# rubengooj/pl-slam

Measured on AMD Instinct MI355X. Metric: stereo pairs/sec (1500 ORB + 200 LBD BF-match), higher is better.
Workload: dtype fp4; 1 GPU; C2: synthetic 752x480 stereo stream, 1500 ORB + 200 LBD per image, ORB+LBD L<->R and prev<->curr, mutual + ratio (StVO::match), then StereoFrame's gates over the L<->R tables (config_kitti.yaml:25-...; mutual=True, distinct_batches_in_rotation=3, stereo_gates=True, kernel=k_scan_sym_mfma_i, mfma_form=0

## Files before the change

plslam_amd/csrc/hamming_mfma_i.hip:

```cpp
#include "mfma_h_common.hpp"

#include <type_traits>


namespace plslam {

namespace {
constexpr uint32_t MI_MAG = FP4_FOUR;
constexpr int MI_DSHIFT = 5;
constexpr uint32_t MI_ACC_BITS = 0x4B000000u + 4096u;
constexpr uint32_t MI_KEY16_MAX = 0x3FFFu;
constexpr uint32_t MI_COL_PENALTY = 0x4000u;
constexpr int MI_SCALE_A = 0, MI_SCALE_B = 0;
constexpr uint32_t MI_NONE16 = 0x7BFFu;
constexpr uint32_t MI_NONE32 = MI_NONE16 * 0x00010001u;
constexpr int MI_RESCAN_BATCH = 2;
constexpr int MI_RESCAN_BATCH16 = 2;
constexpr int MI_VGPRS = 168;
}

#ifdef PLSLAM_MI_PROF
constexpr int MI_PROF_WGS = 65536;
__device__ unsigned long long g_mi_prof[MI_PROF_WGS * 4];
#define PLSLAM_MI_TICK() __builtin_readcyclecounter()
#endif

template <bool DIRECTED>
__global__ void __launch_bounds__(256, 3) __attribute__((amdgpu_num_vgpr(MI_VGPRS / 2)))
k_scan_sym_mfma_i(const SymDesc* __restrict__ syms, const BlockDesc* __restrict__ blocks, int32_t* __restrict__ zero, int nzero, int nblocks)
{
    constexpr int ROWX_STRIDE = 33;
    constexpr int MI_ROW_STRIDE = MH_ROW_STRIDE, MI_TILE_BYTES = MH_TILE_N * MI_ROW_STRIDE;
    constexpr int PARK_OFF = 2 * MI_TILE_BYTES;
    constexpr int SMEM_BYTES = PARK_OFF + 4 * 16 * 64 * 8;
    static_assert(SMEM_BYTES >= 4 * 64 * ROWX_STRIDE * 4, "the transpose must fit");
    __shared__ __attribute__((aligned(16))) uint8_t smem[SMEM_BYTES];
    __shared__ __attribute__((aligned(16))) uint32_t colstage[MH_CGROUP * 256];
    constexpr int RING = 3;
    __shared__ __attribute__((aligned(16))) uint32_t rawring[RING][256];
    uint8_t* const btile = smem;
    u32x2_t* const park = reinterpret_cast<u32x2_t*>(smem + PARK_OFF) + (threadIdx.x >> 6) * (16 * 64) + (threadIdx.x & 63);

#ifdef PLSLAM_MI_PROF
    const unsigned long long prof_t0 = PLSLAM_MI_TICK();
    unsigned long long prof_loop = 0, prof_fin = 0, prof_tl = 0;
#endif
    if (blockIdx.x == 0)
        for (int i = threadIdx.x; i < nzero; i += 256) zero[i] = 0;
    asm volatile("s_setreg_imm32_b32 hwreg(HW_REG_MODE, 6, 2), 3");

    (void)nblocks;
    const int wg = xcd_remap_(blockIdx.x, gridDim.x);
    const BlockDesc bd = blocks[wg];
    if (bd.item < 0) return;
    const SymDesc sd = syms[bd.item];
    const int n1 = sd.n1, n2 = sd.n2;
    const MhLayout L(n2);
    const int ntiles = L.ntiles, nfull = L.nfull, rag_s = L.rag_s;
    const int n2p = (MH_TILE_N * ntiles + 255) & ~255;
    const int tid = threadIdx.x, lane = tid & 63;
    const int w = __builtin_amdgcn_readfirstlane(tid >> 6);
    const int c = lane & 31, g = lane >> 5;
    const gcu32_t araw = (gcu32_t) reinterpret_cast<const uint32_t*>(sd.a);
    const int iw = bd.row0 + 32 * w;

    i32x4 afrag[2][MH_KSTEPS];

    uint32_t gm[16];
#pragma unroll
    for (int s = 0; s < 16; ++s) gm[s] = MI_NONE32;

    u32x16 seed;
#pragma unroll
    for (int r = 0; r < 16; ++r) seed[r] = MI_ACC_BITS + (uint32_t)(16 * g + r);
    asm volatile("" : "+v"(seed));
    const int rest = n2 - (nfull >> 4) * MH_GROUP_ROWS;
    auto lane_lim = [&]() __attribute__((always_inline)) -> int {
        const int cc = (int)(threadIdx.x & 31u), v = rest - rag_s * cc;
        return rag_s == 0 ? 0 : (v < 0 ? 0 : (v > rag_s ? rag_s : v));
    };
    const int lim_part = rag_s ? rest % rag_s : 0;
    const int mask_from = rest - 31 * rag_s < 0 ? 0 : rest - 31 * rag_s;

    const bool block_ragged = bd.row0 + 256 > n1;
    const bool wide_part = !DIRECTED && (sd.flags & 1);
    const gu32_t part = DIRECTED ? (gu32_t) nullptr : (gu32_t) sd.part21 + (size_t)(bd.row0 >> 8) * n2p * (wide_part ? 2 : 1);
    uint32_t* const cstage = colstage + 64 * w;
#pragma unroll
    for (int k = 0; k < 2; ++k) *reinterpret_cast<i32x4*>(colstage + 8 * tid + 4 * k) = i32x4{-1, -1, -1, -1};

    const int ej = tid >> 3, ewd4 = (tid & 7) * 4;
    const PLSLAM_GLOBAL char* const bbytes = (const PLSLAM_GLOBAL char*) sd.b;
    auto load_raw = [&](int t) __attribute__((always_inline)) -> uint32_t {
        const int tc = t < ntiles ? t : ntiles - 1;
        const int gbase = (tc >> 4) * MH_GROUP_ROWS;
        const uint32_t s = tc < nfull ? (uint32_t)MH_GROUP : (uint32_t)rag_s;
        uint32_t row = __umul24((uint32_t)ej, s) + (uint32_t)(tc & 15);
        const uint32_t last = (uint32_t)(n2 - 1 - gbase);
        row = row < last ? row : last;
        return *reinterpret_cast<gcu32_t>(bbytes + (size_t)gbase * 32 + (row * 32u + (uint32_t)ewd4));
    };
    auto load_raw_async = [&](int t, uint32_t slot_b) __attribute__((always_inline)) {
        const int tc = t < ntiles ? t : ntiles - 1;
        const uint32_t s = tc < nfull ? (uint32_t)MH_GROUP : (uint32_t)rag_s;
        const uint32_t first = ((uint32_t)(tc & ~15) << 5) + (uint32_t)(tc & 15);
        uint32_t row = __umul24((uint32_t)ej, s) + first;
        const uint32_t last = (uint32_t)(n2 - 1);
        row = row < last ? row : last;
        const uint32_t voff = row * 32u + (uint32_t)ewd4;
        const uint32_t lds_dst = (uint32_t)(uintptr_t)(&rawring[0][64 * w]) + slot_b;
        asm volatile("s_mov_b32 m0, %2\n\ts_nop 0\n\tglobal_load_lds_dword %0, %1" : : "v"(voff), "s"(bbytes), "s"(lds_dst) : "memory", "m0");
    };
    uint32_t pf32 = 0;
    auto load_raw_async_full = [&](uint32_t slot_b) __attribute__((always_inline)) {
        const uint32_t voff = (uint32_t)(ej * (MH_GROUP * 32) + ewd4) + pf32;
        const uint32_t lds_dst = (uint32_t)(uintptr_t)(&rawring[0][64 * w]) + slot_b;
        asm volatile("s_mov_b32 m0, %2\n\ts_nop 0\n\tglobal_load_lds_dword %0, %1" : : "v"(voff), "s"(bbytes), "s"(lds_dst) : "memory", "m0");
    };
    auto take_raw = [&](uint32_t slot_b) __attribute__((always_inline)) -> uint32_t {
        asm volatile("s_waitcnt vmcnt(2)" ::: "memory");
        return *reinterpret_cast<const uint32_t*>(reinterpret_cast<const uint8_t*>(&rawring[0][0]) + slot_b + (ej * 32 + ewd4));
    };
    auto expand_store = [&](uint32_t raw, int buf, int tn, bool full = false) __attribute__((always_inline)) {
        uint8_t* dst = btile + buf * MI_TILE_BYTES + ej * MI_ROW_STRIDE + ewd4 * 4;
        i32x4 v = expand_dword_fp4<false, MI_MAG>(raw);
        if (!full && tn >= nfull && (tn & 15) >= mask_from) {
            const int vm = (int)(__umul24((uint32_t)rag_s, (uint32_t)ej) + (uint32_t)(tn & 15)) < rest ? -1 : 0;
            v &= i32x4{vm, vm, vm, vm};
        }
        *reinterpret_cast<i32x4*>(dst) = v;
    };

    int wt0 = 0, wt1 = ntiles < MH_WINDOW ? ntiles : MH_WINDOW;
    uint32_t ring_slot = 1024;

    const uint64_t part_u = (uint64_t)(uintptr_t)part;
    const uint64_t part_s = ((uint64_t)(uint32_t)__builtin_amdgcn_readfirstlane((int)(part_u >> 32)) << 32) |
                            (uint32_t)__builtin_amdgcn_readfirstlane((int)(uint32_t)part_u);
    auto combine_columns = [&](int kb) __attribute__((always_inline)) {
        if (DIRECTED) return;
        uint32_t l_;
        asm volatile("v_mbcnt_lo_u32_b32 %0, -1, 0\n\tv_mbcnt_hi_u32_b32 %0, -1, %0" : "=&v"(l_));
        const uint32_t* const src = colstage + 512 * w + (((l_ & 32u) << 3) | (l_ & 31u));
        uint32_t p[8];
#pragma unroll
        for (int v = 0; v < 4; ++v) { p[2 * v] = src[64 * v]; p[2 * v + 1] = src[64 * v + 32]; }
        if (block_ragged) {
#pragma unroll
            for (int q = 0; q < 8; ++q) {
                const int base = bd.row0 + 32 * (q >> 1) + 16 * (q & 1);
                const uint32_t strike = (base >= n1 ? MI_NONE16 : 0u) | (base + 128 >= n1 ? MI_NONE16 << 16 : 0u);
                p[q] = pk_max16(p[q], strike);
            }
        }
        auto pk_merge = [](uint32_t& a0, uint32_t& a1, uint32_t c0, uint32_t c1) {
            const uint32_t m = pk_max16(a0, c0);
            a0 = pk_min16(a0, c0);
            a1 = pk_min16(m, pk_min16(a1, c1));
        };
        uint32_t k0, k1;
        if (!wide_part) {
            uint32_t lo[4], hi[4], enc[4];
#pragma unroll
            for (int q = 0; q < 4; ++q) { lo[q] = pk_min16(p[2 * q], p[2 * q + 1]); hi[q] = pk_max16(p[2 * q], p[2 * q + 1]); }
#pragma unroll
            for (int q = 0; q < 4; ++q) {
                uint32_t t;
                asm("v_pk_add_u16 %0, %1, %2" : "=v"(t) : "v"(lo[q]), "v"((uint32_t)(32 * q) * 0x00010001u));
                asm("v_pk_mad_u16 %0, %1, %2, %3 clamp" : "=v"(enc[q]) : "v"(lo[q] & 0xFFE0FFE0u), "v"(0x00030003u), "v"(t));
            }
            const uint32_t best = pk_min16(pk_min16(enc[0], enc[1]), pk_min16(enc[2], enc[3]));
            pk_merge(lo[0], hi[0], lo[1], hi[1]);
            pk_merge(lo[2], hi[2], lo[3], hi[3]);
            pk_merge(lo[0], hi[0], lo[2], hi[2]);
            const uint32_t e0 = best & 0xFFFFu, u0 = best >> 16, e1 = hi[0] & 0xFFE0u, u1 = (hi[0] >> 16) & 0xFFE0u;
            k0 = e0 + (e0 & 0xFF80u);
            k1 = e1 << 3;
            merge2(k0, k1, u0 + (u0 & 0xFF80u) + 128u, u1 << 3);
        } else {
#pragma unroll
            for (int q = 0; q < 8; ++q) {
                const uint32_t t = p[q] & 0x001F001Fu;
                uint32_t sh;
                asm("v_pk_lshlrev_b16 %0, %1, %2" : "=v"(sh) : "v"(0x00020002u), "v"(p[q] & 0xFFE0FFE0u));
                p[q] = sh | t | ((uint32_t)(q >> 1) << 5) * 0x00010001u;
            }
            uint32_t lo[4], hi[4];
#pragma unroll
            for (int q = 0; q < 4; ++q) { lo[q] = pk_min16(p[2 * q], p[2 * q + 1]); hi[q] = pk_max16(p[2 * q], p[2 * q + 1]); }
            pk_merge(lo[0], hi[0], lo[1], hi[1]);
            pk_merge(lo[2], hi[2], lo[3], hi[3]);
            pk_merge(lo[0], hi[0], lo[2], hi[2]);
            const uint32_t e0 = lo[0] & 0xFFFFu, e1 = hi[0] & 0xFFFFu, u0 = lo[0] >> 16, u1 = hi[0] >> 16;
            k0 = e0 + (e0 & 0xFF80u); k1 = e1 + (e1 & 0xFF80u);
            merge2(k0, k1, u0 + (u0 & 0xFF80u) + 128u, u1 + (u1 & 0xFF80u) + 128u);
        }
        const uint32_t slot4 = (uint32_t)(256 * kb + 64 * w) * 4u;
        if (!wide_part) {
            const uint32_t e = (umin_(k0, 0x1FFFFu) << 9) | umin_(k1 >> 8, 511u);
            PLSLAM_GLOBAL uint32_t* dst = (PLSLAM_GLOBAL uint32_t*)((PLSLAM_GLOBAL char*)(uintptr_t)(part_s + slot4) + 4u * l_);
            __builtin_nontemporal_store(e, dst);
        } else {
            const u32x2_t e = {k0, k1};
            PLSLAM_GLOBAL u32x2_t* dst = (PLSLAM_GLOBAL u32x2_t*)((PLSLAM_GLOBAL char*)(uintptr_t)(part_s + 2u * slot4) + 8u * l_);
            __builtin_nontemporal_store(e, dst);
        }
    };
    auto push_groups = [&gm, &wt0, &park](int t, auto final_tag, u32x2_t* rb) __attribute__((always_inline)) {
        constexpr bool FINAL = decltype(final_tag)::value;
        const uint32_t grp = (uint32_t)(((t - wt0) >> 4) & 3);
        const uint32_t gtag = grp * 0x00010001u;
        uint32_t gtv = gtag;
        asm volatile("" : "+v"(gtv));
        auto retag = [&](uint32_t x) -> uint32_t {
            uint32_t r;
            asm("v_and_or_b32 %0, %1, %2, %3" : "=v"(r) : "v"(x), "s"(0xFFE0FFE0u), "v"(gtv));
            return r;
        };
        if (grp == 0) {
#pragma unroll
            for (int s = 0; s < 16; ++s) {
                const u32x2_t v = {retag(gm[s]), 0xFFFFFFFFu};
                if (FINAL) rb[s] = v;
                else park[s * 64] = v;
                gm[s] = MI_NONE32;
            }
            return;
        }
#pragma unroll
        for (int s = 0; s < 16; ++s) {
            const u32x2_t v = park[s * 64];
            uint32_t b0 = v.x, b1 = v.y;
            pk_push2(b0, b1, retag(gm[s]));
            if (FINAL) rb[s] = u32x2_t{b0, b1};
            else park[s * 64] = u32x2_t{b0, b1};
            gm[s] = MI_NONE32;
        }
    };
    auto finish_columns = [&](int t, uint32_t c0, uint32_t c1) __attribute__((always_inline)) {
        if (DIRECTED) { asm volatile("" ::"v"(c0), "v"(c1)); return; }
        cstage[(t & (MH_CGROUP - 1)) * 256 + lane] = __builtin_amdgcn_perm(c1, c0, 0x05040100u);
    };

#define PLSLAM_MI_EPI2(ACC, MT, Q)                                                                 \
    {                                                                                              \
        asm("v_pk_minimum3_f16 %0, %0, %1, %2 op_sel:[0,0,1] op_sel_hi:[1,1,0]" : "+v"(gm[8 * (MT) + (Q)]) : "v"(ACC[Q]), "v"(ACC[(Q) + 8])); \
        asm("v_pk_minimum3_f16 %0, %0, %1, %2 op_sel:[0,0,1] op_sel_hi:[1,1,0]" : "+v"(gm[8 * (MT) + (Q) + 1]) : "v"(ACC[(Q) + 1]), "v"(ACC[(Q) + 9])); \
        if (!DIRECTED) {    \
            if ((Q) == 0) asm("v_min_f32 %0, %1, %2" : "=v"(cfa) : "v"(ACC[Q]), "v"(ACC[(Q) + 8])); \
            else asm("v_min3_f32 %0, %0, %1, %2" : "+v"(cfa) : "v"(ACC[Q]), "v"(ACC[(Q) + 8]));    \
            asm("v_min3_f32 %0, %0, %1, %2" : "+v"(cfa) : "v"(ACC[(Q) + 1]), "v"(ACC[(Q) + 9]));   \
        }                                                                                          \
        __builtin_amdgcn_sched_barrier(0);                                                         \
    }
#define PLSLAM_MI_MMA(ACC, MT, KS, CIN)                                                            \
    {                                                                                              \
        const i32x8 a8 = {afrag[MT][KS].x, afrag[MT][KS].y, afrag[MT][KS].z, afrag[MT][KS].w, 0, 0, 0, 0}; \
        const i32x8 b8 = {bfr[KS].x, bfr[KS].y, bfr[KS].z, bfr[KS].w, 0, 0, 0, 0};                 \
        ACC = __builtin_amdgcn_mfma_scale_f32_32x32x64_f8f6f4(a8, b8, CIN, 4, 4, 0, MI_SCALE_A, 0, MI_SCALE_B); \
        asm volatile("" : "+v"(ACC));                      \
        __builtin_amdgcn_sched_barrier(0);                                                         \
    }
    f32x16 m1;
    uint32_t cm0_prev = MI_NONE32;
    auto tile_step = [&](int t, auto u_tag, bool with_prev, auto full_tag) __attribute__((always_inline)) {
        constexpr bool FULL = decltype(full_tag)::value;
        constexpr int U = decltype(u_tag)::value;
        __syncthreads();
        const uint8_t* bt = btile + (U & 1) * MI_TILE_BYTES + c * MI_ROW_STRIDE + 16 * g;
        i32x4 bfr[MH_KSTEPS];
#define PLSLAM_MI_READ_B(KS) (*reinterpret_cast<const i32x4*>(bt + 32 * (KS)))
        bfr[0] = PLSLAM_MI_READ_B(0);
        bfr[1] = PLSLAM_MI_READ_B(1);
        if (!FULL && t >= nfull && ((t & 15) == 0 || (t & 15) == lim_part)) {
            const uint32_t pen = lane_lim() == (t & 15) ? MI_COL_PENALTY : 0u;
#pragma unroll
            for (int r = 0; r < 16; ++r) seed[r] += pen;
            asm volatile("" : "+v"(seed));
        }
        const f32x16 cseed = __builtin_bit_cast(f32x16, seed);
        f32x16 m0;
        float cfa = 0.0f;
        auto cf_join = [&]() __attribute__((always_inline)) -> uint32_t { return __builtin_bit_cast(uint32_t, cfa); };
        __builtin_amdgcn_sched_barrier(0);
        if (DIRECTED) asm volatile("s_nop 7"); else asm volatile("s_nop 4");
        __builtin_amdgcn_sched_barrier(0);
        PLSLAM_MI_EPI2(m1, 1, 0) PLSLAM_MI_MMA(m0, 0, 0, cseed)
        bfr[2] = PLSLAM_MI_READ_B(2);
        PLSLAM_MI_EPI2(m1, 1, 2) PLSLAM_MI_MMA(m0, 0, 1, m0)
        bfr[3] = PLSLAM_MI_READ_B(3);
        PLSLAM_MI_EPI2(m1, 1, 4) PLSLAM_MI_MMA(m0, 0, 2, m0)
        const uint32_t raw_next = take_raw(ring_slot);
        PLSLAM_MI_EPI2(m1, 1, 6) PLSLAM_MI_MMA(m0, 0, 3, m0)
        const uint32_t cm1 = cf_join();
        expand_store(raw_next, (U + 1) & 1, t + 1, FULL);
        if (FULL) {
            load_raw_async_full(ring_slot);
            pf32 += (U == 3 && ((t + 5) & 15) == 0) ? (MH_GROUP_ROWS - 15) * 32u : 32u;
        } else {
            load_raw_async(t + 4, ring_slot);
        }
        ring_slot = ring_slot == 2048u ? 0u : ring_slot + 1024u;
        if (with_prev) {
            if (!DIRECTED && U == 1 && ((t - 1) & (MH_CGROUP - 1)) == 0 && t - 9 >= wt0) {
                combine_columns((t - 9) >> 3);
                __syncthreads();
            }
            finish_columns(t - 1, cm0_prev, cm1);
            if (U == 0 && ((t - 1) & (MH_GROUP - 1)) == MH_GROUP - 1) push_groups(t - 1, std::false_type{}, nullptr);
        }
        __builtin_amdgcn_sched_barrier(0);
        asm volatile("v_mfma_f32_32x32x64_f8f6f4 %0, %1, %2, %3 cbsz:4 blgp:4" : "=&v"(m1) : "v"(afrag[1][0]), "v"(bfr[0]), "v"(cseed));
        __builtin_amdgcn_sched_barrier(0);
        PLSLAM_MI_EPI2(m0, 0, 0)
        PLSLAM_MI_MMA(m1, 1, 1, m1)    PLSLAM_MI_EPI2(m0, 0, 2)
        PLSLAM_MI_MMA(m1, 1, 2, m1)    PLSLAM_MI_EPI2(m0, 0, 4)
        PLSLAM_MI_MMA(m1, 1, 3, m1)    PLSLAM_MI_EPI2(m0, 0, 6)
        cm0_prev = cf_join();
    };
    auto epilogue = [&](int t) __attribute__((always_inline)) {
        float cfa = 0.0f;
        asm volatile("s_nop 7\n\ts_nop 7");
        __builtin_amdgcn_sched_barrier(0);
        PLSLAM_MI_EPI2(m1, 1, 0) PLSLAM_MI_EPI2(m1, 1, 2) PLSLAM_MI_EPI2(m1, 1, 4) PLSLAM_MI_EPI2(m1, 1, 6)
        finish_columns(t, cm0_prev, __builtin_bit_cast(uint32_t, cfa));
    };
    auto pipeline = [&](u32x2_t* rb) __attribute__((always_inline)) {
        {
            u32x16 none;
#pragma unroll
            for (int r = 0; r < 16; ++r) asm volatile("v_mov_b32 %0, %1" : "=v"(none[r]) : "s"(MI_NONE32));
            m1 = __builtin_bit_cast(f32x16, none);
        }
        int tb = wt0;
        {
            const int lim = (wt1 < nfull ? wt1 : nfull) - 7;
            pf32 = (((uint32_t)((tb + 4) & ~15) << 5) + (uint32_t)((tb + 4) & 15)) * 32u;
            for (; tb < lim; tb += 4) {
                tile_step(tb, std::integral_constant<int, 0>{}, tb != wt0, std::true_type{});
                tile_step(tb + 1, std::integral_constant<int, 1>{}, true, std::true_type{});
                tile_step(tb + 2, std::integral_constant<int, 2>{}, true, std::true_type{});
                tile_step(tb + 3, std::integral_constant<int, 3>{}, true, std::true_type{});
            }
        }
        for (; tb < wt1; tb += 4) {
            tile_step(tb, std::integral_constant<int, 0>{}, tb != wt0, std::false_type{});
            if (tb + 1 < wt1) tile_step(tb + 1, std::integral_constant<int, 1>{}, true, std::false_type{});
            if (tb + 2 < wt1) tile_step(tb + 2, std::integral_constant<int, 2>{}, true, std::false_type{});
            if (tb + 3 < wt1) tile_step(tb + 3, std::integral_constant<int, 3>{}, true, std::false_type{});
        }
        if (!DIRECTED && ((wt1 - 1) & (MH_CGROUP - 1)) == 0 && wt1 - 9 >= wt0) {
            __syncthreads();
            combine_columns((wt1 - 9) >> 3);
            __syncthreads();
        }
        epilogue(wt1 - 1);
        push_groups(wt1 - 1, std::true_type{}, rb);
    };
#undef PLSLAM_MI_EPI2
#undef PLSLAM_MI_MMA
#undef PLSLAM_MI_READ_B

    auto finish_rows = [&](const u32x2_t* rb) __attribute__((always_inline)) {
        uint32_t* rowx = reinterpret_cast<uint32_t*>(smem) + w * (64 * ROWX_STRIDE);
#pragma unroll
        for (int s = 0; s < 16; ++s) {
            const int lrow = 32 * (s >> 3) + 16 * g + (s & 7);
            rowx[lrow * ROWX_STRIDE + c] = __builtin_amdgcn_perm(rb[s].y, rb[s].x, 0x05040100u);
            rowx[(lrow + 8) * ROWX_STRIDE + c] = __builtin_amdgcn_perm(rb[s].y, rb[s].x, 0x07060302u);
        }
        __builtin_amdgcn_fence(__ATOMIC_RELEASE, "wavefront");
        __builtin_amdgcn_wave_barrier();
        __builtin_amdgcn_fence(__ATOMIC_ACQUIRE, "wavefront");
        uint32_t k0 = 0xFFFFFFFFu, k1 = 0xFFFFFFFFu;
        const uint32_t* mine = rowx + lane * ROWX_STRIDE;
#pragma unroll
        for (int cls = 0; cls < 32; ++cls) {
            uint32_t x;
            asm("v_lshl_or_b32 %0, %1, 16, %2" : "=v"(x) : "v"(mine[cls]), "n"(cls));
            asm("v_med3_u32 %0, %1, %2, %0" : "+v"(k1) : "v"(k0), "v"(x));
            k0 = umin_(k0, x);
        }
        {
            const uint32_t cs = k0 & 31u;
            k1 = umin_(k1, (mine[cs] & 0xFFFF0000u) | cs);
        }
        int row = iw + lane + (lane & 32) * 3;
        asm volatile("" : "+v"(row));
        if (row < n1) {
            const gu2_t out = (gu2_t) reinterpret_cast<u32x2_t*>(sd.keys12) + row;
            const gcu32x4_t ap = (gcu32x4_t)(araw + (size_t)row * 8);
            const u32x4_t a_lo = ap[0], a_hi = ap[1];
            auto group_of = [&](uint32_t k, uint32_t& jbase, uint32_t& cnt) {
                const uint32_t t0 = (uint32_t)wt0 + (((k >> 16) & 3u) << 4);
                const uint32_t s = t0 < (uint32_t)nfull ? (uint32_t)MH_GROUP : (uint32_t)rag_s;
                jbase = (t0 >> 4) * MH_GROUP_ROWS + s * (k & 0xFFFFu);
                cnt = s;
            };
            auto rescan = [&](uint32_t jbase, uint32_t cnt, uint32_t& best, uint32_t& second) {
                best = second = KEY_NONE;
                const uint32_t left = (uint32_t)n2 - jbase;
                const uint32_t nvalid = cnt < left ? cnt : left;
                const PLSLAM_GLOBAL char* const rbp = bbytes + (size_t)jbase * 32;
#pragma unroll
                for (int k0_ = 0; k0_ < MH_GROUP; k0_ += MI_RESCAN_BATCH) {
                    u32x4_t bl[MI_RESCAN_BATCH], bh[MI_RESCAN_BATCH];
#pragma unroll
                    for (int q = 0; q < MI_RESCAN_BATCH; ++q) {
                        const uint32_t kk = (uint32_t)(k0_ + q) < nvalid ? (uint32_t)(k0_ + q) : nvalid - 1u;
                        const gcu32x4_t bp = (gcu32x4_t)(rbp + kk * 32u);
                        bl[q] = bp[0];
                        bh[q] = bp[1];
                    }
#pragma unroll
                    for (int q = 0; q < MI_RESCAN_BATCH; ++q) {
                        const uint32_t d = hamming256(a_lo, a_hi, bl[q], bh[q]);
                        const uint32_t cand = (uint32_t)(k0_ + q) < nvalid ? ((d << KEY_IDX_BITS) | (jbase + (uint32_t)(k0_ + q))) : KEY_NONE;
                        second = umin_(second, umax_(best, cand));
                        best = umin_(best, cand);
                    }
                }
            };
            auto rescan16 = [&](uint32_t jb, uint32_t& best, uint32_t& second) {
                uint32_t bk = 0xFFFFFFFFu, sk = 0xFFFFFFFFu;
                const PLSLAM_GLOBAL char* const rbp = bbytes + (size_t)jb * 32;
                constexpr int RB = MI_RESCAN_BATCH16;
#pragma unroll
                for (int k0_ = 0; k0_ < 16; k0_ += RB) {
                    u32x4_t bl[RB], bh[RB];
#pragma unroll
                    for (int q = 0; q < RB; ++q) {
                        const gcu32x4_t bp = (gcu32x4_t)(rbp + (k0_ + q) * 32);
                        bl[q] = bp[0];
                        bh[q] = bp[1];
                    }
#pragma unroll
                    for (int q = 0; q < RB; ++q) {
                        const uint32_t d = hamming256(a_lo, a_hi, bl[q], bh[q]);
                        uint32_t x;
                        asm("v_lshl_or_b32 %0, %1, 4, %2" : "=v"(x) : "v"(d), "n"(k0_ + q));
                        asm("v_med3_u32 %0, %1, %2, %0" : "+v"(sk) : "v"(bk), "v"(x));
                        bk = umin_(bk, x);
                    }
                }
                best = ((bk >> 4) << KEY_IDX_BITS) | (jb + (bk & 15u));
                second = ((sk >> 4) << KEY_IDX_BITS) | (jb + (sk & 15u));
            };
            uint32_t r0 = KEY_NONE, r1 = KEY_NONE;
            if ((k0 >> 16) <= MI_KEY16_MAX) {
                uint32_t jb, cnt, in2;
                group_of(k0, jb, cnt);
                const uint32_t jsh = jb + 16u <= (uint32_t)n2 ? jb : (uint32_t)n2 - 16u;
                const bool guarded = n2 < 16 || jsh < (uint32_t)wt0 * MH_TILE_N;
                if (__builtin_amdgcn_ballot_w64(guarded) == 0) rescan16(jsh, r0, in2);
                else rescan(jb, cnt, r0, in2);
                if ((k1 >> 16) <= MI_KEY16_MAX) {
                    uint32_t jb1, cnt1;
                    group_of(k1, jb1, cnt1);
                    uint32_t o1 = ((k1 >> (16 + MI_DSHIFT)) << KEY_IDX_BITS) | jb1;
                    if ((sd.flags & 1) && (o1 >> KEY_IDX_BITS) <= (in2 >> KEY_IDX_BITS)) {
                        uint32_t b1, s1;
                        rescan(jb1, cnt1, b1, s1);
                        o1 = b1;
                    }
                    r1 = umin_(in2, o1);
                } else {
                    r1 = in2;
                }
            }
            if (wt0 > 0) {
                const u32x2_t prev = *out;
                merge2(r0, r1, prev.x, prev.y);
            }
            *out = u32x2_t{r0, r1};
        }
        __builtin_amdgcn_fence(__ATOMIC_RELEASE, "wavefront");
        __builtin_amdgcn_wave_barrier();
    };

    uint32_t raw_first = load_raw(0);
    load_raw_async(1, 1024);
    load_raw_async(2, 2048);
    load_raw_async(3, 0);
#pragma unroll
    for (int mt = 0; mt < 2; ++mt) {
        const int row = bd.row0 + 128 * mt + 32 * w + 16 * ((c >> 2) & 1) + (c & 3) + 4 * (c >> 3);
        const int rrow = row < n1 ? row : n1 - 1;
        const gcu32_t p = araw + (size_t)rrow * 8 + g;
#pragma unroll
        for (int ks = 0; ks < MH_KSTEPS; ++ks) afrag[mt][ks] = expand_dword_fp4<true, MI_MAG>(p[2 * ks]);
    }

#ifdef PLSLAM_MI_PROF
    const unsigned long long prof_t1 = PLSLAM_MI_TICK();
#endif
    for (;;) {
#ifdef PLSLAM_MI_PROF
        prof_tl = PLSLAM_MI_TICK();
#endif
        expand_store(raw_first, 0, wt0);
        ring_slot = 1024;
        u32x2_t rb[16];
        __builtin_amdgcn_s_setprio(1);
        pipeline(rb);
        __builtin_amdgcn_s_setprio(0);
#ifdef PLSLAM_MI_PROF
        { const unsigned long long t = PLSLAM_MI_TICK(); prof_loop += t - prof_tl; prof_tl = t; }
#endif
        __syncthreads();
        combine_columns((wt1 - 1) >> 3);
        finish_rows(rb);
#ifdef PLSLAM_MI_PROF
        prof_fin += PLSLAM_MI_TICK() - prof_tl;
#endif
        if (wt1 == ntiles) break;
        __syncthreads();
        wt0 = wt1;
        wt1 = ntiles < wt0 + MH_WINDOW ? ntiles : wt0 + MH_WINDOW;
        raw_first = load_raw(wt0);
        load_raw_async(wt0 + 1, 1024);
        load_raw_async(wt0 + 2, 2048);
        load_raw_async(wt0 + 3, 0);
    }
#ifdef PLSLAM_MI_PROF
    if (threadIdx.x == 0 && blockIdx.x < MI_PROF_WGS) {
        g_mi_prof[4 * blockIdx.x + 0] = prof_t1 - prof_t0;
        g_mi_prof[4 * blockIdx.x + 1] = prof_loop;
        g_mi_prof[4 * blockIdx.x + 2] = prof_fin;
        g_mi_prof[4 * blockIdx.x + 3] = ((unsigned long long)ntiles << 40) | (PLSLAM_MI_TICK() - prof_t0);
    }
#endif
}

#ifdef PLSLAM_MI_PROF
extern "C" int plslam_debug_k1i_profile(unsigned long long* out, int nwg)
{
    if (nwg > MI_PROF_WGS) nwg = MI_PROF_WGS;
    return hipMemcpyFromSymbol(out, HIP_SYMBOL(g_mi_prof), sizeof(unsigned long long) * 4 * (size_t)nwg) == hipSuccess ? nwg : -1;
}
#endif

int launch_scan_sym_mfma_i(const SymDesc* d_sym, const BlockDesc* d_blocks, int nblocks, int32_t* d_zero, int nzero,
                           bool directed, hipStream_t s)
{
    if (nblocks <= 0) return PLSLAM_OK;
    if (directed) hipLaunchKernelGGL((k_scan_sym_mfma_i<true>), dim3(nblocks), dim3(256), 0, s, d_sym, d_blocks, d_zero, nzero, nblocks);
    else hipLaunchKernelGGL((k_scan_sym_mfma_i<false>), dim3(nblocks), dim3(256), 0, s, d_sym, d_blocks, d_zero, nzero, nblocks);
    PLSLAM_HIP_CHECK(hipGetLastError());
    return PLSLAM_OK;
}

}
```

Baseline: 1.671 million stereo pairs/s.

## Cooperative quad rescan16: split 16-candidate rescan across four lanes with DPP merge

The 16-candidate rescan is restructured so each quad of lanes works together. Every lane loads the A descriptors of all four rows in its quad and scans a strided quarter of each row's 16 B candidates. Partial best/second keys are merged with quad DPP swaps, and the B loads are software-pipelined through a rotating buffer of depth four. The aim is more coalesced B loads and hidden memory latency, in exchange for extra A loads, extra registers, and the whole wave running the fast path even on inactive rows.

```diff
diff --git a/plslam_amd/csrc/hamming_mfma_i.hip b/plslam_amd/csrc/hamming_mfma_i.hip
--- a/plslam_amd/csrc/hamming_mfma_i.hip
+++ b/plslam_amd/csrc/hamming_mfma_i.hip
@@ -15,7 +15,8 @@
 constexpr uint32_t MI_NONE16 = 0x7BFFu;
 constexpr uint32_t MI_NONE32 = MI_NONE16 * 0x00010001u;
 constexpr int MI_RESCAN_BATCH = 2;
-constexpr int MI_RESCAN_BATCH16 = 2;
+constexpr int MI_RESCAN_G = 4;
+constexpr int MI_RESCAN_DEPTH = 4;
 constexpr int MI_VGPRS = 168;
 }
 
@@ -387,17 +388,92 @@
         }
         int row = iw + lane + (lane & 32) * 3;
         asm volatile("" : "+v"(row));
-        if (row < n1) {
+        const bool live = row < n1;
+        auto group_of = [&](uint32_t k, uint32_t& jbase, uint32_t& cnt) {
+            const uint32_t t0 = (uint32_t)wt0 + (((k >> 16) & 3u) << 4);
+            const uint32_t s = t0 < (uint32_t)nfull ? (uint32_t)MH_GROUP : (uint32_t)rag_s;
+            jbase = (t0 >> 4) * MH_GROUP_ROWS + s * (k & 0xFFFFu);
+            cnt = s;
+        };
+        constexpr int RG = MI_RESCAN_G, RSLICES = 16 / RG, RD = MI_RESCAN_DEPTH, RUNITS = RG * RSLICES * 2;
+        static_assert(RG == 4 && RD >= 1 && RD <= RUNITS, "the DPP steps below are those of a quad");
+        auto dpp = [](uint32_t x, auto ctrl_tag) __attribute__((always_inline)) -> uint32_t {
+            return (uint32_t)__builtin_amdgcn_update_dpp(0, (int)x, decltype(ctrl_tag)::value, 0xF, 0xF, true);
+        };
+        constexpr int DPP_XOR1 = 0xB1, DPP_XOR2 = 0x4E;
+        auto rescan16 = [&](uint32_t jb, int row_, uint32_t& best, uint32_t& second) {
+            const uint32_t m = (uint32_t)lane & (uint32_t)(RG - 1);
+            const int grow0 = row_ - (int)m;
+            u32x4_t av[RG][2];
+            uint32_t boff[RG];
+#pragma unroll
+            for (int r = 0; r < RG; ++r) {
+                const int rr = grow0 + r < n1 ? grow0 + r : n1 - 1;
+                const gcu32x4_t ap = (gcu32x4_t)(araw + (size_t)rr * 8);
+                av[r][0] = ap[0];
+                av[r][1] = ap[1];
+                const uint32_t jr = r == 0   ? dpp(jb, std::integral_constant<int, 0x00>{})
+                                    : r == 1 ? dpp(jb, std::integral_constant<int, 0x55>{})
+                                    : r == 2 ? dpp(jb, std::integral_constant<int, 0xAA>{})
+                                             : dpp(jb, std::integral_constant<int, 0xFF>{});
+                boff[r] = (jr + m) * 32u;
+            }
+            uint32_t rbk = 0xFFFFFFFFu, rsk = 0xFFFFFFFFu;
+            uint32_t bk = 0xFFFFFFFFu, sk = 0xFFFFFFFFu, d = 0;
+            auto load_unit = [&](int u) __attribute__((always_inline)) -> u32x4_t {
+                const int r = u / (RSLICES * 2), sl = (u / 2) % RSLICES, h = u % 2;
+                return *(gcu32x4_t)(bbytes + boff[r] + (sl * (RG * 32) + 16 * h));
+            };
+            u32x4_t bv[RD];
+#pragma unroll
+            for (int q = 0; q < RD; ++q) bv[q] = load_unit(q);
+            __builtin_amdgcn_sched_barrier(0);
+#pragma unroll
+            for (int u = 0; u < RUNITS; ++u) {
+                const int r = u / (RSLICES * 2), sl = (u / 2) % RSLICES, h = u % 2;
+                const u32x4_t x4 = av[r][h] ^ bv[u % RD];
+                if (u + RD < RUNITS) bv[u % RD] = load_unit(u + RD);
+                d = bcnt_acc_(x4.x, h == 0 ? 0u : d);
+                d = bcnt_acc_(x4.y, d);
+                d = bcnt_acc_(x4.z, d);
+                d = bcnt_acc_(x4.w, d);
+                if (h == 1) {
+                    uint32_t x;
+                    asm("v_lshl_or_b32 %0, %1, 4, %2" : "=v"(x) : "v"(d), "n"(sl * RG));
+                    if (sl == 0) {
+                        bk = x;
+                        sk = 0xFFFFFFFFu;
+                    } else {
+                        asm("v_med3_u32 %0, %1, %2, %0" : "+v"(sk) : "v"(bk), "v"(x));
+                        bk = umin_(bk, x);
+                    }
+                    if (sl == RSLICES - 1) {
+                        bk |= m;
+                        sk |= m;
+                        merge2(bk, sk, dpp(bk, std::integral_constant<int, DPP_XOR1>{}), dpp(sk, std::integral_constant<int, DPP_XOR1>{}));
+                        merge2(bk, sk, dpp(bk, std::integral_constant<int, DPP_XOR2>{}), dpp(sk, std::integral_constant<int, DPP_XOR2>{}));
+                        rbk = m == (uint32_t)r ? bk : rbk;
+                        rsk = m == (uint32_t)r ? sk : rsk;
+                    }
+                }
+                __builtin_amdgcn_sched_barrier(0);
+            }
+            best = ((rbk >> 4) << KEY_IDX_BITS) | (jb + (rbk & 15u));
+            second = ((rsk >> 4) << KEY_IDX_BITS) | (jb + (rsk & 15u));
+        };
+        uint32_t jb0 = 0, cnt0 = 0;
+        group_of(k0, jb0, cnt0);
+        const bool have0 = live && (k0 >> 16) <= MI_KEY16_MAX;
+        const uint32_t jsh = jb0 + 16u <= (uint32_t)n2 ? jb0 : (uint32_t)n2 - 16u;
+        const bool guarded = have0 && (n2 < 16 || jsh < (uint32_t)wt0 * MH_TILE_N);
+        const bool fast = n2 >= 16 && __builtin_amdgcn_ballot_w64(guarded) == 0;
+        uint32_t f0 = KEY_NONE, f1 = KEY_NONE;
+        if (fast) rescan16(have0 ? jsh : 0u, row, f0, f1);
+        if (live) {
             const gu2_t out = (gu2_t) reinterpret_cast<u32x2_t*>(sd.keys12) + row;
-            const gcu32x4_t ap = (gcu32x4_t)(araw + (size_t)row * 8);
-            const u32x4_t a_lo = ap[0], a_hi = ap[1];
-            auto group_of = [&](uint32_t k, uint32_t& jbase, uint32_t& cnt) {
-                const uint32_t t0 = (uint32_t)wt0 + (((k >> 16) & 3u) << 4);
-                const uint32_t s = t0 < (uint32_t)nfull ? (uint32_t)MH_GROUP : (uint32_t)rag_s;
-                jbase = (t0 >> 4) * MH_GROUP_ROWS + s * (k & 0xFFFFu);
-                cnt = s;
-            };
             auto rescan = [&](uint32_t jbase, uint32_t cnt, uint32_t& best, uint32_t& second) {
+                const gcu32x4_t ap = (gcu32x4_t)(araw + (size_t)row * 8);
+                const u32x4_t a_lo = ap[0], a_hi = ap[1];
                 best = second = KEY_NONE;
                 const uint32_t left = (uint32_t)n2 - jbase;
                 const uint32_t nvalid = cnt < left ? cnt : left;
@@ -421,39 +497,11 @@
                     }
                 }
             };
-            auto rescan16 = [&](uint32_t jb, uint32_t& best, uint32_t& second) {
-                uint32_t bk = 0xFFFFFFFFu, sk = 0xFFFFFFFFu;
-                const PLSLAM_GLOBAL char* const rbp = bbytes + (size_t)jb * 32;
-                constexpr int RB = MI_RESCAN_BATCH16;
-#pragma unroll
-                for (int k0_ = 0; k0_ < 16; k0_ += RB) {
-                    u32x4_t bl[RB], bh[RB];
-#pragma unroll
-                    for (int q = 0; q < RB; ++q) {
-                        const gcu32x4_t bp = (gcu32x4_t)(rbp + (k0_ + q) * 32);
-                        bl[q] = bp[0];
-                        bh[q] = bp[1];
-                    }
-#pragma unroll
-                    for (int q = 0; q < RB; ++q) {
-                        const uint32_t d = hamming256(a_lo, a_hi, bl[q], bh[q]);
-                        uint32_t x;
-                        asm("v_lshl_or_b32 %0, %1, 4, %2" : "=v"(x) : "v"(d), "n"(k0_ + q));
-                        asm("v_med3_u32 %0, %1, %2, %0" : "+v"(sk) : "v"(bk), "v"(x));
-                        bk = umin_(bk, x);
-                    }
-                }
-                best = ((bk >> 4) << KEY_IDX_BITS) | (jb + (bk & 15u));
-                second = ((sk >> 4) << KEY_IDX_BITS) | (jb + (sk & 15u));
-            };
             uint32_t r0 = KEY_NONE, r1 = KEY_NONE;
-            if ((k0 >> 16) <= MI_KEY16_MAX) {
-                uint32_t jb, cnt, in2;
-                group_of(k0, jb, cnt);
-                const uint32_t jsh = jb + 16u <= (uint32_t)n2 ? jb : (uint32_t)n2 - 16u;
-                const bool guarded = n2 < 16 || jsh < (uint32_t)wt0 * MH_TILE_N;
-                if (__builtin_amdgcn_ballot_w64(guarded) == 0) rescan16(jsh, r0, in2);
-                else rescan(jb, cnt, r0, in2);
+            if (have0) {
+                uint32_t in2 = f1;
+                r0 = f0;
+                if (!fast) rescan(jb0, cnt0, r0, in2);
                 if ((k1 >> 16) <= MI_KEY16_MAX) {
                     uint32_t jb1, cnt1;
                     group_of(k1, jb1, cnt1);
```

New measurement: 1.683 million stereo pairs/s (median of 6 runs). No clear change (+0.7%).
